# supernomad/quantum

Measured on AMD Instinct MI355X. Metric: AES-256-GCM seal+unseal GiB/s (device-resident packets) at 1/2/4/8 MI355X, higher is better.
Workload: dtype u8

## Files before the change

### quantum_amd/csrc/gcm_internal.h

```cpp
#pragma once
#include <hip/hip_runtime.h>

#include <sched.h>

#include <mutex>
#include <stdint.h>
#include <vector>

#include "../../include/qgcm.h"
#include "nonce_rng.h"
#include "one_fit.h"

namespace qgcm {

constexpr uint32_t kTeBytes = 65536;
constexpr uint32_t kGhBytes = 8192;
constexpr uint32_t kRkWords = 128;
constexpr uint32_t kGhEntries = 4608;
constexpr uint32_t kGhH = 0, kGhH4 = 512, kGhH2 = 1024, kGhH3 = 1536, kGhH5 = 2048;
constexpr uint32_t kGhH8 = 2560, kGhH16 = 3072, kGhH32 = 3584, kGhH64 = 4096;

struct Batch {
    uint8_t *arena;
    const qgcm_desc *descs;
    const uint32_t *worklist;
    const uint8_t *nonces;
    uint8_t *status;
    const uint32_t *rk_table;
    const uint4 *gh_table;
    const uint32_t *te;
    const uint8_t *key_valid;
    uint64_t stride;
    uint32_t uniform_len;
    uint32_t uniform_key;
    uint32_t n;
    uint32_t n_items;
    uint32_t aad_len;
    uint32_t max_keys;
    uint32_t *tile_counter;
    const uint32_t *tile_keys;
    const uint2 *runs;
    uint32_t *run_next;
    const uint32_t *nruns;
    const uint32_t *tile_list;
    const uint32_t *n_list;
    uint8_t *done;
    const uint4 *pw_table;
    uint32_t pw_keys;
    uint32_t *pool;
    uint32_t *pool_done;
    uint32_t pool_gen;
// ... 192 lines not shown
```

### quantum_amd/csrc/gcm_kernels.hip

```cpp
#include <hip/hip_runtime.h>
#include <stdint.h>

#include <algorithm>

#include "gcm_internal.h"

namespace qgcm {

typedef __attribute__((address_space(3))) uint32_t lds_u32;
typedef uint32_t u32x4 __attribute__((ext_vector_type(4)));
typedef __attribute__((address_space(3))) u32x4 lds_u128;

struct __attribute__((aligned(4))) W4 {
    uint32_t x, y, z, w;
};

#ifndef QGCM_NT_DATA
#define QGCM_NT_DATA 0
#endif
typedef uint32_t u32x4u __attribute__((ext_vector_type(4), aligned(4)));
__device__ __forceinline__ W4 load_block(const W4 *p) {
    if constexpr ((QGCM_NT_DATA & 1) != 0) {
        const u32x4u v = __builtin_nontemporal_load(reinterpret_cast<const u32x4u *>(p));
        return W4{v.x, v.y, v.z, v.w};
    }
    return *p;
}
__device__ __forceinline__ void store_block(W4 *p, const W4 &v) {
    if constexpr ((QGCM_NT_DATA & 2) != 0) {
        __builtin_nontemporal_store(u32x4u{v.x, v.y, v.z, v.w}, reinterpret_cast<u32x4u *>(p));
        return;
    }
    *p = v;
}

__device__ __forceinline__ uint32_t perm(uint32_t s0, uint32_t s1, uint32_t sel) {
// ... 135 lines not shown
    const uint32_t x = lo ^ c.x3;
    const uint32_t t0 = c.K0 ^ rot16(lds32(((x << 8) | t.lb) + kB + 128u));
    s0 = c.U0 ^ t.t0(t0, 0);
    s1 = c.U1 ^ rot16(t.t1(t0, 3));
    s2 = c.U2 ^ rot16(t.t0(t0, 2));
    s3 = c.U3 ^ t.t1(t0, 1);
#pragma unroll
    for (int r = 3; r < 14; ++r) round_full(s0, s1, s2, s3, k, r, t);
    round_last(s0, s1, s2, s3, k, t);
}
__device__ __forceinline__ void ctr_block(const Ctr &c, uint32_t lo, const Keys &k, uint32_t lb, uint32_t &s0,
                                          uint32_t &s1, uint32_t &s2, uint32_t &s3) {
    ctr_block_t<TT0, 0>(c, lo, k, TT0{lb, 0}, s0, s1, s2, s3);
}

template <bool kFence>
__device__ __forceinline__ void ghash_mul(uint32_t &y0, uint32_t &y1, uint32_t &y2, uint32_t &y3, uint32_t gb);

struct Tab2 {
    Keys kk;
    TT<0, true> t;
    __device__ __forceinline__ void setup(Ctr &c, uint32_t n0, uint32_t n1, uint32_t n2, uint32_t hi) const {
        ctr_setup(c, n0, n1, n2, hi, kk, t);
    }
    __device__ __forceinline__ void block(const Ctr &c, uint32_t lo, uint32_t &k0, uint32_t &k1, uint32_t &k2,
                                          uint32_t &k3) const {
        ctr_block_t<TT<0, true>, 0>(c, lo, kk, t, k0, k1, k2, k3);
    }
    __device__ __forceinline__ void ghash(uint32_t &y0, uint32_t &y1, uint32_t &y2, uint32_t &y3, uint32_t gb) const {
        ghash_mul<true>(y0, y1, y2, y3, gb);
    }
};

constexpr uint32_t kG5Windows = 26;
constexpr uint32_t kG5Bytes = kG5Windows * 512;

template <int kI>
__device__ __forceinline__ uint32_t g5_addr(const uint32_t (&y)[4], uint32_t mf8) {
    constexpr int p = 5 * kI, w = p >> 5, o = p & 31;
    uint32_t x;
    if constexpr (o > 27 && w < 3)
        x = __builtin_amdgcn_alignbit(y[w + 1], y[w], o - 3);
    else if constexpr (o > 3)
        x = y[w] >> (o - 3);
    else if constexpr (o < 3)
        x = y[w] << (3 - o);
    else
        x = y[w];
    return x & mf8;
}

template <int kLo, int kHi>
__device__ __forceinline__ void g5_chunk(const uint32_t (&y)[4], uint32_t mf8, uint32_t &a0, uint32_t &a1,
                                         uint32_t &a2, uint32_t &a3) {
    if constexpr (kLo < kHi) {
        if constexpr (QGCM_GH_PRIO > 0) __builtin_amdgcn_s_setprio(QGCM_GH_PRIO);
        const uint32_t x = g5_addr<kLo>(y, mf8);
        const u32x2 h0 = lds64(x + kLo * 512u), h1 = lds64(x + kLo * 512u + 256u);
        if constexpr (kLo + 1 < kHi) {
            const uint32_t x2 = g5_addr<kLo + 1>(y, mf8);
            const u32x2 l0 = lds64(x2 + (kLo + 1) * 512u), l1 = lds64(x2 + (kLo + 1) * 512u + 256u);
            if constexpr (QGCM_GH_PRIO > 0) __builtin_amdgcn_s_setprio(0);
            a0 = xor3(a0, h0.x, l0.x);
            a1 = xor3(a1, h0.y, l0.y);
            a2 = xor3(a2, h1.x, l1.x);
            a3 = xor3(a3, h1.y, l1.y);
            g5_chunk<kLo + 2, kHi>(y, mf8, a0, a1, a2, a3);
        } else {
            if constexpr (QGCM_GH_PRIO > 0) __builtin_amdgcn_s_setprio(0);
            a0 ^= h0.x;
            a1 ^= h0.y;
            a2 ^= h1.x;
            a3 ^= h1.y;
        }
    }
}

__device__ __forceinline__ void ghash_mul5(uint32_t &y0, uint32_t &y1, uint32_t &y2, uint32_t &y3, uint32_t mf8) {
    const uint32_t y[4] = {y0, y1, y2, y3};
    uint32_t a0 = 0, a1 = 0, a2 = 0, a3 = 0;
    g5_chunk<0, 7>(y, mf8, a0, a1, a2, a3);
    asm volatile("" : "+v"(a0), "+v"(a1), "+v"(a2), "+v"(a3)::"memory");
    g5_chunk<7, 13>(y, mf8, a0, a1, a2, a3);
    asm volatile("" : "+v"(a0), "+v"(a1), "+v"(a2), "+v"(a3)::"memory");
    g5_chunk<13, 20>(y, mf8, a0, a1, a2, a3);
    asm volatile("" : "+v"(a0), "+v"(a1), "+v"(a2), "+v"(a3)::"memory");
    g5_chunk<20, 26>(y, mf8, a0, a1, a2, a3);
    y0 = a0;
    y1 = a1;
    y2 = a2;
    y3 = a3;
}

__device__ __forceinline__ void g5_fill(const uint4 *__restrict__ comb4, uint32_t tid, uint32_t nthreads) {
    for (uint32_t e = tid; e < kG5Windows * 32u; e += nthreads) {
        const uint32_t i = e >> 5, v = e & 31u;
        uint4 c[5];
#pragma unroll
        for (uint32_t j = 0; j < 5; ++j) {
            const uint32_t t = 5 * i + j, tt = t < 128u ? t : 127u;
            const uint32_t vv = (((v >> j) & 1u) && t < 128u) ? (1u << (tt & 3u)) : 0u;
            c[j] = comb4[16u * (2u * (tt >> 3) + ((tt & 7u) < 4u ? 1u : 0u)) + vv];
        }
        uint32_t a0 = 0, a1 = 0, a2 = 0, a3 = 0;
#pragma unroll
        for (uint32_t j = 0; j < 5; ++j) {
            a0 ^= c[j].x;
            a1 ^= c[j].y;
            a2 ^= c[j].z;
            a3 ^= c[j].w;
        }
        *(lds_u64 *)(size_t)(512u * i + 8u * v) = u32x2{a0, a1};
        *(lds_u64 *)(size_t)(512u * i + 256u + 8u * v) = u32x2{a2, a3};
    }
}

struct Tab2F {
    Keys kk;
    TT<kG5Bytes, true> t;
    uint32_t mf8;
    __device__ __forceinline__ void setup(Ctr &c, uint32_t n0, uint32_t n1, uint32_t n2, uint32_t hi) const {
        ctr_setup(c, n0, n1, n2, hi, kk, t);
    }
    __device__ __forceinline__ void block(const Ctr &c, uint32_t lo, uint32_t &k0, uint32_t &k1, uint32_t &k2,
                                          uint32_t &k3) const {
        ctr_block_t<TT<kG5Bytes, true>, kG5Bytes>(c, lo, kk, t, k0, k1, k2, k3);
    }
    __device__ __forceinline__ void ghash(uint32_t &y0, uint32_t &y1, uint32_t &y2, uint32_t &y3, uint32_t) const {
        ghash_mul5(y0, y1, y2, y3, mf8);
    }
};

__device__ __forceinline__ uint32_t vreg(uint32_t x) {
    asm volatile("" : "+v"(x));
    return x;
}

template <bool kFence = true>
__device__ __forceinline__ void ghash_mul(uint32_t &y0, uint32_t &y1, uint32_t &y2, uint32_t &y3, uint32_t gb) {
    uint32_t a0 = 0, a1 = 0, a2 = 0, a3 = 0;
    const uint32_t yw[4] = {y0, y1, y2, y3};
#pragma unroll
    for (int w = 0; w < 4; ++w) {
        const uint32_t hi = yw[w] & 0xf0f0f0f0u;
        const uint32_t lo = (yw[w] << 4) & 0xf0f0f0f0u;
#pragma unroll
        for (int k = 0; k < 4; ++k) {
            const int j = 4 * w + k;
            const uint4 th = lds128(perm(gb, hi, 0x0c060500u | k) + (2 * j) * 256);
            const uint4 tl = lds128(perm(gb, lo, 0x0c060500u | k) + (2 * j + 1) * 256);
            a0 = xor3(a0, th.x, tl.x);
            a1 = xor3(a1, th.y, tl.y);
            a2 = xor3(a2, th.z, tl.z);
            a3 = xor3(a3, th.w, tl.w);
        }
        if constexpr (kFence) asm volatile("" : "+v"(a0), "+v"(a1), "+v"(a2), "+v"(a3)::"memory");
    }
    y0 = a0;
    y1 = a1;
    y2 = a2;
    y3 = a3;
}
// ... 232 lines not shown
    e2 = quad_xor(e2);
    e3 = quad_xor(e3);
    const uint32_t t0 = z0 ^ e0, t1 = z1 ^ e1, t2 = z2 ^ e2, t3 = z3 ^ e3;
    const uint32_t owner = r ? (nfull & 3u) : 0u;
    if (kSeal) {
        if (m == owner) {
            write_tail(data, L, t0, t1, t2, t3, n0, n1, n2, prefix);
            if (b.status) b.status[pkt] = 1;
        }
    } else {
        read_tag(data, L, g0, g1, g2, g3);
        const bool ok = ((t0 ^ g0) | (t1 ^ g1) | (t2 ^ g2) | (t3 ^ g3)) == 0;
        if (!ok) {
            for (uint32_t bi = m; bi < nfull; bi += 4) {
                const W4 zz = {0, 0, 0, 0};
                *reinterpret_cast<W4 *>(data + 16u * bi) = zz;
            }
            if (r && m == owner) {
                uint32_t *bw = reinterpret_cast<uint32_t *>(data + 16u * nfull);
                for (uint32_t w = 0; w < (r >> 2); ++w) bw[w] = 0;
                store_bytes(data + 16u * nfull + (r & ~3u), 0, r & 3u);
            }
        }
        if (b.status && m == 0) b.status[pkt] = ok ? 1 : 0;
    }
}

#ifndef QGCM_TILE_POOL
#define QGCM_TILE_POOL 4
#endif
#ifndef QGCM_TAIL_EIGHTHS
#define QGCM_TAIL_EIGHTHS 4
#endif
constexpr uint32_t kPoolCtr = kG5Bytes + kTeBytes;

#ifdef QGCM_QUAD_STATS
__device__ unsigned long long g_quad_stats[4096 * 8];
#endif

template <bool kDesc>
constexpr int quad_waves() { return kDesc ? 12 : 16; }
template <bool kDesc>
constexpr int quad_wpe() { return kDesc ? 3 : 8; }

template <bool kSeal, bool kDesc>
__global__ void __launch_bounds__(quad_waves<kDesc>() * 64) __attribute__((amdgpu_waves_per_eu(quad_wpe<kDesc>(),
                                                                                                  quad_wpe<kDesc>())))
gcm_quad_kernel(Batch b, const uint32_t *__restrict__ rk_table) {
    constexpr uint32_t kW = quad_waves<kDesc>();
    constexpr uint32_t kT = kW * 64;
    constexpr uint32_t kTeBase = kDesc ? 0u : kG5Bytes;
    const uint32_t lane = threadIdx.x & 63u;
    const uint32_t wave = threadIdx.x >> 6;
    const uint32_t m = lane & 3u;
    const uint32_t qd = lane >> 2;
    if (kDesc && b.tile_list && __builtin_amdgcn_readfirstlane(*b.n_list) == 0) return;

    for (uint32_t i = threadIdx.x; i < kTeBytes / 4; i += kT) {
        const uint32_t x = i >> 6, slot = i & 63u;
        lds_st32(kTeBase + 4 * i, b.te[(slot >> 5) * 256u + x]);
    }
    if constexpr (!kDesc) g5_fill(b.gh_table + (size_t)b.uniform_key * kGhEntries + kGhH4, threadIdx.x, kT);
    if constexpr (!kDesc && QGCM_TILE_POOL) {
        if (threadIdx.x == 0) lds_st32(kPoolCtr, kW);
    }
#if QGCM_TILE_POOL == 4
    if constexpr (!kDesc) {
        if (threadIdx.x == 0) lds_st32(kPoolCtr + 12, 0u);
    }
#endif
    __syncthreads();

    const uint32_t lb = (lane & 31u) << 2;
    const uint32_t m8 = vreg(0x0000ff00u), mf8 = vreg(0x000000f8u);
    const uint32_t gH4 = kDesc ? kTeBytes + wave * kGhBytes : 0u;
    uint32_t cur_key = kDesc ? 0xffffffffu : b.uniform_key;
    const uint32_t ntiles = kDesc ? (b.tile_list ? *b.n_list : b.n_items >> 4) : ((b.n + 15) >> 4);

#ifdef QGCM_QUAD_STATS
    unsigned long long *qs = g_quad_stats + (size_t)blockIdx.x * 8u;
    uint32_t qs_tiles = 0;
    if (!kDesc && threadIdx.x == 0) {
        qs[0] = wall_clock64();
        qs[4] = __builtin_amdgcn_s_getreg((31 << 11) | 20);
        qs[5] = __builtin_amdgcn_s_getreg((31 << 11) | 4);
    }
#endif
#ifdef QGCM_QUAD_STATS
#define QS_TILE() ++qs_tiles
#define QS_END()                                                  \
    do {                                                          \
        if (!kDesc && lane == 0) {                                \
            const unsigned long long t_ = wall_clock64();         \
            atomicMax(&qs[1], t_);                                \
            atomicAdd(&qs[2], t_);                                \
            atomicAdd(&qs[3], (unsigned long long)qs_tiles);      \
            atomicMax(&qs[6], (1ull << 62) - t_);                 \
        }                                                         \
    } while (0)
#else
#define QS_TILE() do { } while (0)
#define QS_END() do { } while (0)
#endif
#if QGCM_TILE_POOL == 4
    uint32_t sidx = 0xffffffffu, tail0 = 0;
    if constexpr (!kDesc) {
        const uint32_t rows = ntiles / (gridDim.x * kW);
// ... 52 lines not shown
            pkt = tile * 16u + qd;
            L = b.uniform_len;
            asm volatile("" : "+s"(L));
            valid = pkt < b.n;
            if (!kSeal) {
                if (L < (uint32_t)QGCM_OVERHEAD) valid = false;
                L -= QGCM_OVERHEAD;
            }
            off = (uint64_t)pkt * b.stride;
            if constexpr (QGCM_TILE_POOL) {
                uint32_t i = 0;
                if (lane == 0) i = __atomic_fetch_add((lds_u32 *)(size_t)kPoolCtr, 1u, __ATOMIC_RELAXED);
                i = __builtin_amdgcn_readfirstlane(i);
                tile = blockIdx.x * kW + (i % kW) + (i / kW) * gridDim.x * kW;
#if QGCM_TILE_POOL == 4
                if (i >= sidx) {
                    uint32_t c = 0;
                    if (lane == 0) c = atomicAdd(b.pool, 1u);
                    tile = tail0 + __builtin_amdgcn_readfirstlane(c);
                }
#endif
            } else {
                tile += gridDim.x * kW;
            }
            if (!valid) {
                if (!kSeal && b.status && pkt < b.n && m == 0) b.status[pkt] = 0;
                continue;
            }
        }
        const Keys kk = {rk_table + (size_t)wkey * kRkWords, rk_table + (size_t)wkey * kRkWords + 64};
        if constexpr (kDesc) {
            quad_packet<kSeal>(b, Tab2{kk, {lb, m8}}, pkt, off, L, wkey, m, gH4);
        } else {
            quad_packet<kSeal>(b, Tab2F{kk, {lb, m8}, mf8}, pkt, off, L, wkey, m, gH4);
        }
        QS_TILE();
    }
    QS_END();
#if QGCM_TILE_POOL == 4
    if constexpr (!kDesc) {
        if (b.pool) {
            uint32_t last = 0;
            if (lane == 0 && __atomic_fetch_add((lds_u32 *)(size_t)(kPoolCtr + 12), 1u, __ATOMIC_RELAXED) == kW - 1) {
                __threadfence();
                last = atomicAdd(b.pool + kPoolDoneWord, 1u) == gridDim.x - 1u ? 1u : 0u;
            }
            if (lane == 0 && last) {
                __threadfence();
                b.pool[0] = 0;
                b.pool[kPoolDoneWord] = 0;
                __threadfence_system();
                __hip_atomic_store(b.pool_done, b.pool_gen, __ATOMIC_RELEASE, __HIP_MEMORY_SCOPE_SYSTEM);
            }
        }
    }
#endif
}
#undef QS_TILE
#undef QS_END

#ifdef QGCM_QUAD_STATS
extern "C" int qgcm_debug_quad_stats(unsigned long long *out, int n, int reset) {
    if (n > 4096 * 8) n = 4096 * 8;
    if (hipMemcpyFromSymbol(out, HIP_SYMBOL(g_quad_stats), (size_t)n * 8) != hipSuccess) return -1;
    if (reset) {
        static unsigned long long zero[4096 * 8];
        if (hipMemcpyToSymbol(HIP_SYMBOL(g_quad_stats), zero, sizeof(zero)) != hipSuccess) return -1;
    }
    return 0;
}
#endif

constexpr uint32_t kSegCtl = kG5Bytes + kTeBytes;
constexpr uint32_t kSegLds = kSegCtl + 16u;
constexpr uint32_t kSegDone = 0xffffffffu;

__device__ __forceinline__ volatile lds_u32 *seg_ctl(uint32_t i) { return (volatile lds_u32 *)(size_t)(kSegCtl + 4u * i); }

template <class P>
__device__ __forceinline__ uint32_t wave_lower_bound(uint32_t lo, uint32_t hi, uint32_t lane, P pred) {
    while (hi - lo > 63u) {
        const uint32_t step = (hi - lo + 62u) / 63u;
        const uint32_t p = min(lo + lane * step, hi);
        const uint64_t msk = __ballot(pred(p));
        const uint32_t f = (uint32_t)__ffsll((unsigned long long)msk) - 1u;
        if (f == 0) return lo;
        const uint32_t nlo = lo + (f - 1u) * step + 1u, nhi = min(lo + f * step, hi);
        lo = nlo;
        hi = nhi;
    }
    const uint64_t msk = __ballot(pred(min(lo + lane, hi)));
    return lo + (uint32_t)__ffsll((unsigned long long)msk) - 1u;
}

#ifdef QGCM_SEG_STATS
__device__ unsigned long long g_seg_stats[4096 * 16];
#define SEG_STAT_ADD(i, v) \
    do { if (lane == 0) atomicAdd(&g_seg_stats[blockIdx.x * 16u + (i)], (unsigned long long)(v)); } while (0)
#define SEG_NOW() wall_clock64()
#else
#define SEG_STAT_ADD(i, v) do { } while (0)
#define SEG_NOW() 0ull
#endif

#ifndef QGCM_SEG_START
#define QGCM_SEG_START 1
// ... 43 lines not shown
            for (uint32_t j = 0; j < 4 && found == kSegDone; ++j) {
                const uint64_t msk = __ballot(left[j]);
                if (msk) found = __builtin_amdgcn_readfirstlane(__shfl(idx[j], (int)__ffsll((unsigned long long)msk) - 1));
            }
            if (found != kSegDone) break;
        }
    }
    uint32_t key = kSegDone;
    if (found != kSegDone) {
        r = found;
        key = b.tile_keys[b.runs[found].x];
    }
    if (lane == 0) {
        *seg_ctl(0) = found;
        *seg_ctl(1) = key;
    }
}

#ifndef QGCM_SEG_CLAIM
#define QGCM_SEG_CLAIM 1
#endif

template <bool kSeal>
__global__ void __launch_bounds__(1024) __attribute__((amdgpu_waves_per_eu(8, 8)))
gcm_seg_kernel(Batch b, const uint32_t *__restrict__ rk_table) {
    constexpr uint32_t kT = 1024;
    const uint32_t lane = threadIdx.x & 63u;
    const uint32_t wave = threadIdx.x >> 6;
    const uint32_t m = lane & 3u;
    const uint32_t qd = lane >> 2;
    if (__builtin_amdgcn_readfirstlane(*b.nruns) == 0) return;
    for (uint32_t i = threadIdx.x; i < kTeBytes / 4; i += kT) {
        const uint32_t x = i >> 6, slot = i & 63u;
        lds_st32(kG5Bytes + 4 * i, b.te[(slot >> 5) * 256u + x]);
    }
    const uint32_t lb = (lane & 31u) << 2;
    const uint32_t m8 = vreg(0x0000ff00u), mf8 = vreg(0x000000f8u);
    const uint32_t ntiles = b.n_items >> 4;
    uint32_t table_key = kSegDone;
    uint32_t r = 0, nruns = 0;
    bool helping = false;
    if (wave == 0) {
        nruns = *b.nruns;
        const uint32_t t = (uint32_t)((uint64_t)ntiles * blockIdx.x / gridDim.x);
        const uint32_t i = wave_lower_bound(0u, nruns, lane, [&](uint32_t j) { return j == nruns || b.runs[j].x > t; });
        r = i ? i - 1u : 0u;
        SEG_STAT_ADD(6, r);
        SEG_STAT_ADD(8, __builtin_amdgcn_s_getreg((31 << 11) | 20));
        SEG_STAT_ADD(9, __builtin_amdgcn_s_getreg((31 << 11) | 4));
    }
    __syncthreads();
    [[maybe_unused]] unsigned long long t_idle = SEG_NOW();
    if (wave == 0) SEG_STAT_ADD(2, t_idle);
    [[maybe_unused]] uint32_t ntile_stat = 0;
    for (;;) {
        if (wave == 0) {
            [[maybe_unused]] const unsigned long long t0 = SEG_NOW();
            seg_next_phase(b, r, nruns, helping, lane);
            SEG_STAT_ADD(7, SEG_NOW() - t0);
        }
        __syncthreads();
        if (wave == 0) SEG_STAT_ADD(0, 1);
        const uint32_t run = __builtin_amdgcn_readfirstlane(*seg_ctl(0));
        const uint32_t key = __builtin_amdgcn_readfirstlane(*seg_ctl(1));
        if (run == kSegDone) break;
        if (key != table_key) {
            g5_fill(b.gh_table + (size_t)key * kGhEntries + kGhH4, threadIdx.x, kT);
            table_key = key;
            __syncthreads();
        }
        [[maybe_unused]] const unsigned long long t_busy = SEG_NOW();
        SEG_STAT_ADD(4, t_busy - t_idle);
        const uint2 rt = b.runs[run];
        const Tab2F e3 = {{rk_table + (size_t)key * kRkWords, rk_table + (size_t)key * kRkWords + 64}, {lb, m8}, mf8};
        for (uint32_t t = 0, left = 0;; ++t, --left) {
            if (left == 0) {
                uint32_t nx = 0;
                if (lane == 0) nx = atomicAdd(b.run_next + run, (uint32_t)QGCM_SEG_CLAIM);
                t = rt.x + __builtin_amdgcn_readfirstlane(__shfl(nx, 0));
                left = QGCM_SEG_CLAIM;
            }
            if (t >= rt.y) break;
            const uint32_t pkt = b.worklist[t * 16u + qd];
            if (pkt != 0xffffffffu) {
                const qgcm_desc dsc = b.descs[pkt];
                const uint32_t L = kSeal ? dsc.len : dsc.len - QGCM_OVERHEAD;
                quad_packet<kSeal, Tab2F>(b, e3, pkt, dsc.offset, L, key, m, 0u);
            }
            ++ntile_stat;
        }
        t_idle = SEG_NOW();
        SEG_STAT_ADD(5, t_idle - t_busy);
        __syncthreads();
    }
    SEG_STAT_ADD(1, ntile_stat);
    if (wave == 0) SEG_STAT_ADD(3, SEG_NOW());
}

#ifdef QGCM_SEG_STATS
extern "C" int qgcm_debug_seg_stats(unsigned long long *out, int n, int reset) {
    if (n > 4096 * 16) n = 4096 * 16;
    if (hipMemcpyFromSymbol(out, HIP_SYMBOL(g_seg_stats), (size_t)n * 8) != hipSuccess) return -1;
    if (reset) {
        static unsigned long long zero[4096 * 16];
        if (hipMemcpyToSymbol(HIP_SYMBOL(g_seg_stats), zero, sizeof(zero)) != hipSuccess) return -1;
    }
    return 0;
}
#endif

constexpr uint32_t kOneThreads = 512;
constexpr uint32_t kOneTabs = 7;
constexpr uint32_t kOneBuf = kTeBytes + kOneTabs * kGhBytes;
constexpr uint32_t kOneScratch = kOneBuf + kOneCap;
constexpr uint32_t kOneX = kOneScratch + 64;
constexpr uint32_t kOneLds = kOneX + 2048;
constexpr uint32_t kOneSliceMax = kOneThreads / 4;
static_assert(kOneLds <= 160u * 1024u, "gfx950 LDS is 160 KiB per workgroup");
#ifdef QGCM_RES_TRACE
constexpr uint32_t kResTrace = ((kOneLds + 15u) & ~15u) + 16;
// ... 746 lines not shown
    if (b.aad_len > 4 && (b.n != 1 || b.descs || !one_fits_launch(b.uniform_len, seal, b.aad_len)))
        return hipErrorInvalidValue;
    if (!b.descs) {
        const uint64_t stage = (4ull + b.uniform_len + (seal ? QGCM_OVERHEAD : 0) + 15) & ~15ull;
        if ((b.n > 1 && (b.stride < stage || (b.stride & 15))) || stage > kOneCap - 16 ||
            (!seal && b.uniform_len < QGCM_OVERHEAD))
            return hipErrorInvalidValue;
    }
    void *args[] = {const_cast<Batch *>(&b), const_cast<uint32_t **>(&b.rk_table)};
    const void *k = seal ? reinterpret_cast<const void *>(&gcm_one_kernel<true>)
                         : reinterpret_cast<const void *>(&gcm_one_kernel<false>);
    return hipLaunchKernel(k, dim3(b.n), dim3(kOneThreads), args, kOneLds, s);
}

struct Variant {
    const void *seal, *open;
    int waves;
    uint32_t lds;
    int wgs_per_cu;
    bool desc;
    int complement;
};

static Variant g_variants[3];
static int variant_slot(int v) {
    return v == kVariantUniform ? 0 : v == kVariantDescWave ? 1 : v == kVariantDescQuad ? 2 : -1;
}

static const void *nonce_kernel_of(NonceDest dest);

hipError_t init_kernels() {
    g_variants[0] = Variant{reinterpret_cast<const void *>(&gcm_quad_kernel<true, false>),
                                          reinterpret_cast<const void *>(&gcm_quad_kernel<false, false>),
                                          quad_waves<false>(), kG5Bytes + kTeBytes + 16u,
                                          quad_wpe<false>() * 4 / quad_waves<false>(), false, -1};
    g_variants[1] = Variant{reinterpret_cast<const void *>(&gcm_quad_kernel<true, true>),
                                           reinterpret_cast<const void *>(&gcm_quad_kernel<false, true>),
                                           quad_waves<true>(), kTeBytes + (uint32_t)quad_waves<true>() * kGhBytes,
                                           1, true, -1};
    g_variants[2] = Variant{reinterpret_cast<const void *>(&gcm_seg_kernel<true>),
                                           reinterpret_cast<const void *>(&gcm_seg_kernel<false>), 16, kSegLds, 2, true,
                                           kVariantDescWave};
    for (const Variant &v : g_variants) {
        if (!v.seal) continue;
        for (const void *k : {v.seal, v.open}) {
            hipFuncAttributes a;
            hipError_t e = hipFuncGetAttributes(&a, k);
            if (e != hipSuccess) return e;
            if (a.sharedSizeBytes != 0) return hipErrorInvalidKernelFile;
            e = hipFuncSetAttribute(k, hipFuncAttributeMaxDynamicSharedMemorySize, v.lds);
            if (e != hipSuccess) return e;
        }
    }
    for (const void *k : {reinterpret_cast<const void *>(&gcm_one_kernel<true>),
                          reinterpret_cast<const void *>(&gcm_one_kernel<false>),
                          reinterpret_cast<const void *>(&gcm_resident_kernel)}) {
        hipFuncAttributes a;
        hipError_t e = hipFuncGetAttributes(&a, k);
        if (e != hipSuccess) return e;
        if (a.sharedSizeBytes != 0) return hipErrorInvalidKernelFile;
        e = hipFuncSetAttribute(k, hipFuncAttributeMaxDynamicSharedMemorySize,
                                k == reinterpret_cast<const void *>(&gcm_resident_kernel) ? kResLds : kOneLds);
        if (e != hipSuccess) return e;
    }
    for (NonceDest d : {kNonceArray, kNonceUniform, kNonceDescs}) {
        const void *k = nonce_kernel_of(d);
        hipFuncAttributes a;
// ... 17 lines not shown
    if (!variant_valid(variant)) return hipErrorInvalidValue;
    const Variant &v = g_variants[variant_slot(variant)];
    void *args[] = {const_cast<Batch *>(&b), const_cast<uint32_t **>(&b.rk_table)};
    return hipLaunchKernel(seal ? v.seal : v.open, dim3(grid), dim3(v.waves * 64), args, v.lds, s);
}

__device__ __forceinline__ uint8_t xt(uint8_t a) { return (uint8_t)((a << 1) ^ ((a & 0x80) ? 0x1b : 0)); }

__device__ inline void shift_x(uint8_t v[16]) {
    const int lsb = v[15] & 1;
    for (int j = 15; j > 0; --j) v[j] = (uint8_t)((v[j] >> 1) | (v[j - 1] << 7));
    v[0] >>= 1;
    if (lsb) v[0] ^= 0xe1;
}
__device__ inline uint4 pack16(const uint8_t v[16]) {
    uint4 w;
    w.x = v[0] | v[1] << 8 | v[2] << 16 | (uint32_t)v[3] << 24;
    w.y = v[4] | v[5] << 8 | v[6] << 16 | (uint32_t)v[7] << 24;
    w.z = v[8] | v[9] << 8 | v[10] << 16 | (uint32_t)v[11] << 24;
    w.w = v[12] | v[13] << 8 | v[14] << 16 | (uint32_t)v[15] << 24;
    return w;
}
__device__ inline void gf128_mul_bytes(const uint8_t X[16], const uint8_t Y[16], uint8_t Z[16]) {
    uint8_t z[16] = {0}, v[16];
    for (int i = 0; i < 16; ++i) v[i] = Y[i];
    for (int i = 0; i < 128; ++i) {
        if ((X[i >> 3] >> (7 - (i & 7))) & 1)
            for (int j = 0; j < 16; ++j) z[j] ^= v[j];
        shift_x(v);
    }
    for (int i = 0; i < 16; ++i) Z[i] = z[i];
}

__global__ void __launch_bounds__(256) key_setup_kernel(const uint8_t *keys, uint32_t first, uint32_t *rk_table,
                                                        uint4 *gh_table, const uint8_t *sbox_g) {
    __shared__ uint8_t sbox[256];
    __shared__ uint8_t rkb[240];
    constexpr int kT = kGhEntries / 512;
    __shared__ uint8_t hp[kT][16];
    __shared__ uint4 pw[kT][128];
    const uint32_t kidx = blockIdx.x;
    const uint8_t *key = keys + 32u * kidx;
    sbox[threadIdx.x] = sbox_g[threadIdx.x];
    __syncthreads();
    if (threadIdx.x == 0) {
        for (int i = 0; i < 32; ++i) rkb[i] = key[i];
        uint8_t rcon = 1;
        for (int i = 8; i < 60; ++i) {
            uint8_t t[4] = {rkb[4 * i - 4], rkb[4 * i - 3], rkb[4 * i - 2], rkb[4 * i - 1]};
            if (i % 8 == 0) {
                const uint8_t t0 = t[0];
                t[0] = sbox[t[1]] ^ rcon;
                t[1] = sbox[t[2]];
                t[2] = sbox[t[3]];
                t[3] = sbox[t0];
                rcon = xt(rcon);
            } else if (i % 8 == 4) {
                for (int j = 0; j < 4; ++j) t[j] = sbox[t[j]];
            }
            for (int j = 0; j < 4; ++j) rkb[4 * i + j] = rkb[4 * i - 32 + j] ^ t[j];
        }
        uint8_t s[16], u[16];
        for (int i = 0; i < 16; ++i) s[i] = rkb[i];
        for (int round = 1; round <= 14; ++round) {
            for (int c = 0; c < 4; ++c)
                for (int r = 0; r < 4; ++r) u[r + 4 * c] = sbox[s[r + 4 * ((c + r) & 3)]];
            if (round != 14) {
                for (int c = 0; c < 4; ++c) {
                    const uint8_t a0 = u[4 * c], a1 = u[4 * c + 1], a2 = u[4 * c + 2], a3 = u[4 * c + 3];
                    const uint8_t all = a0 ^ a1 ^ a2 ^ a3;
                    s[4 * c + 0] = a0 ^ all ^ xt(a0 ^ a1);
// ... 2 lines not shown
                    s[4 * c + 3] = a3 ^ all ^ xt(a3 ^ a0);
                }
            } else {
                for (int i = 0; i < 16; ++i) s[i] = u[i];
            }
            for (int i = 0; i < 16; ++i) s[i] ^= rkb[16 * round + i];
        }
        for (int i = 0; i < 16; ++i) hp[0][i] = s[i];
        gf128_mul_bytes(s, s, hp[2]);
        gf128_mul_bytes(hp[2], s, hp[3]);
        gf128_mul_bytes(hp[2], hp[2], hp[1]);
        gf128_mul_bytes(hp[1], s, hp[4]);
        for (int t = 5; t < kT; ++t) gf128_mul_bytes(hp[t == 5 ? 1 : t - 1], hp[t == 5 ? 1 : t - 1], hp[t]);
    }
    __syncthreads();
    if (threadIdx.x < kT) {
        uint8_t v[16];
        for (int i = 0; i < 16; ++i) v[i] = hp[threadIdx.x][i];
        for (int i = 0; i < 128; ++i) {
            pw[threadIdx.x][i] = pack16(v);
            shift_x(v);
        }
    }
    __syncthreads();
    const uint32_t slot = first + kidx;
    if (threadIdx.x < 64) {
        const int i = threadIdx.x;
        const uint32_t w = i < 60 ? (rkb[4 * i] | rkb[4 * i + 1] << 8 | rkb[4 * i + 2] << 16 |
                                     (uint32_t)rkb[4 * i + 3] << 24)
                                  : 0u;
        rk_table[(size_t)slot * kRkWords + i] = w;
        rk_table[(size_t)slot * kRkWords + 64 + i] = (w << 16) | (w >> 16);
    }
    for (uint32_t e = threadIdx.x; e < kGhEntries; e += 256) {
        const uint32_t p = (e & 511u) >> 4, v = e & 15u;
        const uint4 *src = pw[e >> 9];
        uint4 acc = {0, 0, 0, 0};
        for (int k = 0; k < 4; ++k) {
            if ((v >> (3 - k)) & 1u) {
                const uint4 t = src[4 * p + k];
                acc.x ^= t.x;
                acc.y ^= t.y;
                acc.z ^= t.z;
                acc.w ^= t.w;
            }
        }
        gh_table[(size_t)slot * kGhEntries + e] = acc;
    }
}

hipError_t launch_key_setup(const uint8_t *d_keys, uint32_t first, uint32_t count, uint32_t *rk_table,
                            uint4 *gh_table, const uint8_t *d_sbox, hipStream_t s) {
    if (count == 0) return hipSuccess;
    hipLaunchKernelGGL(key_setup_kernel, dim3(count), dim3(256), 0, s, d_keys, first, rk_table, gh_table, d_sbox);
    return hipGetLastError();
}

__global__ void __launch_bounds__(256) pw_setup_kernel(uint32_t first, const uint4 *gh_table, uint4 *pw,
                                                       uint32_t pw_keys) {
    __shared__ uint8_t hp[kPwPowers][16];
    __shared__ uint4 xs[16][128];
    const uint32_t slot = first + blockIdx.x, tid = threadIdx.x;
    if (slot >= pw_keys) return;
    if (tid == 0) {
        const uint4 h = gh_table[(size_t)slot * kGhEntries + kGhH + 8];
        const uint32_t w[4] = {h.x, h.y, h.z, h.w};
        for (int i = 0; i < 16; ++i) hp[0][i] = (uint8_t)(w[i >> 2] >> (8 * (i & 3)));
    }
    __syncthreads();
    for (uint32_t span = 1; span < kPwPowers; span <<= 1) {
        if (tid >= span && tid < 2 * span && tid < kPwPowers) gf128_mul_bytes(hp[tid - span], hp[span - 1], hp[tid]);
        __syncthreads();
    }
    for (uint32_t b0 = 0; b0 < kPwPowers; b0 += 16) {
        {
            const uint32_t j = tid >> 4, i0 = 8 * (tid & 15u);
            uint8_t v[16];
            for (int i = 0; i < 16; ++i) v[i] = hp[b0 + j][i];
            for (uint32_t i = 0; i < i0; ++i) shift_x(v);
            for (uint32_t i = 0; i < 8; ++i) {
// ... 211 lines not shown
```

### quantum_amd/csrc/qgcm_api.cpp

```cpp
#include <hip/hip_runtime.h>
#include <errno.h>
#include <stdint.h>
#include <stdio.h>
#include <stdlib.h>
#include <string.h>
#include <sys/random.h>

#include <algorithm>
#include <atomic>
#include <chrono>
#include <memory>
#include <future>
#include <map>
#include <mutex>
#include <thread>
#include <vector>

#include "../../include/qgcm.h"
#include "chain_claim.h"
#include "gcm_internal.h"
#include "kdf_core.h"

using namespace qgcm;

// ... 979 lines not shown
    const PeerPublics pp{priv_key, priv_salt, pub_keys, pub_salts};
    return derive_install_runs(ctx, &run, 1, count, nullptr, nullptr, &pp);
}

int qgcm_ecdh_stats(const qgcm_ctx *ctx, uint64_t *out, int n) {
    if (!ctx || !out || n < 0) return -1;
    const int m = std::min(n, 3);
    for (int i = 0; i < m; ++i) out[i] = ctx->ecdh_stats[i].load(std::memory_order_relaxed);
    return m;
}

int qgcm_kdf_stats(const qgcm_ctx *ctx, uint64_t *out, int n) {
    if (!ctx || !out || n < 0) return -1;
    const int m = std::min(n, 4);
    for (int i = 0; i < m; ++i) out[i] = ctx->kdf_stats[i].load(std::memory_order_relaxed);
    return m;
}

int qgcm_clear_keys(qgcm_ctx *ctx, uint32_t first_idx, uint32_t count) {
    if (!ctx) return QGCM_E_ARG;
    if ((uint64_t)first_idx + count > ctx->max_keys) return QGCM_E_KEY;
    if (count == 0) return QGCM_OK;
    if (hipSetDevice(ctx->device) != hipSuccess) return QGCM_E_HIP;
    std::lock_guard<std::mutex> io(ctx->io_mu);
    hipStream_t s = ctx->pipe[1];
    std::lock_guard<std::mutex> res_lk(ctx->res_mu);
    Resident *res = ctx->res.load(std::memory_order_acquire);
    (void)resident_pause(res);
    {
        std::lock_guard<std::mutex> g(ctx->key_mu);
        for (uint32_t i = 0; i < count; ++i) __atomic_store_n(&ctx->key_set[first_idx + i], (uint8_t)0, __ATOMIC_RELEASE);
    }
    int rc = QGCM_OK;
    if (hipMemsetAsync(ctx->d_key_valid + first_idx, 0, count, s) != hipSuccess || hipStreamSynchronize(s) != hipSuccess)
        rc = QGCM_E_HIP;
    resident_resume(res);
    return rc;
}

int qgcm_seal_batch(qgcm_ctx *ctx, uint8_t *d_arena, const qgcm_desc *d_descs, uint32_t n, const uint8_t *d_nonces,
                    uint32_t aad_len, uint8_t *d_status, void *stream) {
    return run_descs(ctx, true, d_arena, d_descs, n, d_nonces, aad_len, d_status, (hipStream_t)stream);
}

int qgcm_open_batch(qgcm_ctx *ctx, uint8_t *d_arena, const qgcm_desc *d_descs, uint32_t n, uint32_t aad_len,
                    uint8_t *d_status, void *stream) {
    return run_descs(ctx, false, d_arena, d_descs, n, nullptr, aad_len, d_status, (hipStream_t)stream);
}

int qgcm_seal_uniform(qgcm_ctx *ctx, uint8_t *d_arena, uint64_t stride, uint32_t n, uint32_t len, uint32_t key_idx,
                      const uint8_t *d_nonces, uint32_t aad_len, uint8_t *d_status, void *stream) {
    return run_uniform(ctx, true, d_arena, stride, n, len, key_idx, d_nonces, aad_len, d_status, (hipStream_t)stream);
}

int qgcm_open_uniform(qgcm_ctx *ctx, uint8_t *d_arena, uint64_t stride, uint32_t n, uint32_t len, uint32_t key_idx,
                      uint32_t aad_len, uint8_t *d_status, void *stream) {
    if (n > QGCM_MAX_BATCH) return QGCM_E_ARG;
    if (len < QGCM_OVERHEAD && n) {
        if (!ctx) return QGCM_E_ARG;
        if (d_status) {
            if (hipSetDevice(ctx->device) != hipSuccess) return QGCM_E_HIP;
            return hip_fail(hipMemsetAsync(d_status, 0, n, (hipStream_t)stream));
        }
        return QGCM_OK;
    }
    return run_uniform(ctx, false, d_arena, stride, n, len, key_idx, nullptr, aad_len, d_status, (hipStream_t)stream);
}
// ... 686 lines not shown
```

Measured before the change: 875.8.

## Serve upper GHASH 5-bit comb windows from global rows via buffer loads

Key setup now precomputes the 5-bit comb GHASH rows per key into the global gh_table. The uniform quad kernel then reads the top QGCM_GH_L1 windows (default 2) with buffer loads instead of LDS, interleaving those loads with the LDS lookups. This shrinks the LDS table, which may raise occupancy, and moves part of the lookup traffic to the L1/global path. In exchange each key's table grows by 13 KB, setup does more work, and clear_keys must also zero the extra rows.

```diff
diff --git a/quantum_amd/csrc/g5_comb.h b/quantum_amd/csrc/g5_comb.h
--- /dev/null
+++ b/quantum_amd/csrc/g5_comb.h
@@ -0,0 +1,30 @@
+#pragma once
+#include <stdint.h>
+
+#if defined(__HIPCC__) || defined(__CUDACC__)
+#define QGCM_G5_HD __host__ __device__
+#else
+#define QGCM_G5_HD
+#endif
+
+namespace qgcm {
+
+constexpr uint32_t kG5Windows = 26;
+constexpr uint32_t kG5Rows = kG5Windows * 32;
+
+QGCM_G5_HD constexpr uint32_t g5_bit_entry(uint32_t t) {
+    return 16u * (2u * (t >> 3) + ((t & 7u) < 4u ? 1u : 0u)) + (1u << (t & 3u));
+}
+
+QGCM_G5_HD constexpr uint32_t g5_term(uint32_t i, uint32_t v, uint32_t j) {
+    const uint32_t t = 5u * i + j, tt = t < 128u ? t : 127u;
+    return (((v >> j) & 1u) && t < 128u) ? g5_bit_entry(tt) : (g5_bit_entry(tt) & ~15u);
+}
+
+QGCM_G5_HD constexpr uint32_t g5_l1_first(uint32_t k) { return k >= 6u ? kG5Windows - k : 20u; }
+QGCM_G5_HD constexpr bool g5_in_l1(uint32_t i, uint32_t k) { return i >= g5_l1_first(k) && i < g5_l1_first(k) + k; }
+QGCM_G5_HD constexpr uint32_t g5_lds_slot(uint32_t i, uint32_t k) { return i < g5_l1_first(k) ? i : i - k; }
+QGCM_G5_HD constexpr uint32_t g5_lds_window(uint32_t slot, uint32_t k) { return slot < g5_l1_first(k) ? slot : slot + k; }
+QGCM_G5_HD constexpr uint32_t g5_lds_bytes(uint32_t k) { return (kG5Windows - k) * 512u; }
+
+}
diff --git a/quantum_amd/csrc/gcm_internal.h b/quantum_amd/csrc/gcm_internal.h
--- a/quantum_amd/csrc/gcm_internal.h
+++ b/quantum_amd/csrc/gcm_internal.h
@@ -8,6 +8,7 @@
 #include <vector>
 
 #include "../../include/qgcm.h"
+#include "g5_comb.h"
 #include "nonce_rng.h"
 #include "one_fit.h"
 
@@ -16,7 +17,9 @@
 constexpr uint32_t kTeBytes = 65536;
 constexpr uint32_t kGhBytes = 8192;
 constexpr uint32_t kRkWords = 128;
-constexpr uint32_t kGhEntries = 4608;
+constexpr uint32_t kGhComb = 4608;
+constexpr uint32_t kGhG5 = kGhComb;
+constexpr uint32_t kGhEntries = kGhComb + kG5Rows;
 constexpr uint32_t kGhH = 0, kGhH4 = 512, kGhH2 = 1024, kGhH3 = 1536, kGhH5 = 2048;
 constexpr uint32_t kGhH8 = 2560, kGhH16 = 3072, kGhH32 = 3584, kGhH64 = 4096;
 
diff --git a/quantum_amd/csrc/gcm_kernels.hip b/quantum_amd/csrc/gcm_kernels.hip
--- a/quantum_amd/csrc/gcm_kernels.hip
+++ b/quantum_amd/csrc/gcm_kernels.hip
@@ -2,6 +2,7 @@
 #include <stdint.h>
 
 #include <algorithm>
+#include <utility>
 
 #include "gcm_internal.h"
 
@@ -203,8 +204,64 @@
     }
 };
 
-constexpr uint32_t kG5Windows = 26;
-constexpr uint32_t kG5Bytes = kG5Windows * 512;
+#ifndef QGCM_GH_L1
+#define QGCM_GH_L1 2
+#endif
+#ifndef QGCM_GH_L1_SEG
+#define QGCM_GH_L1_SEG 0
+#endif
+static_assert(QGCM_GH_L1 >= 0 && QGCM_GH_L1 <= 12 && QGCM_GH_L1_SEG >= 0 && QGCM_GH_L1_SEG <= 12,
+              "windows served from the global rows: the upper windows, at most 12");
+constexpr uint32_t kGhL1 = QGCM_GH_L1, kGhL1Seg = QGCM_GH_L1_SEG;
+
+struct G5Rows {
+    __amdgpu_buffer_rsrc_t rsrc;
+};
+template <uint32_t kL1>
+__device__ __forceinline__ G5Rows g5_rows(const uint4 *gh_key) {
+    if constexpr (kL1 == 0) return G5Rows{};
+    const uint4 *rows = gh_key + kGhG5 + 32u * g5_l1_first(kL1);
+    return G5Rows{__builtin_amdgcn_make_buffer_rsrc(const_cast<uint4 *>(rows), 0, (int)(kL1 * 512u), 0x00020000)};
+}
+
+template <int kI>
+__device__ __forceinline__ uint32_t g5_row(const uint32_t (&y)[4]) {
+    constexpr int p = 5 * kI, w = p >> 5, o = p & 31;
+    uint32_t x;
+    if constexpr (o > 27 && w < 3)
+        x = __builtin_amdgcn_alignbit(y[w + 1], y[w], o - 4);
+    else if constexpr (o > 4)
+        x = y[w] >> (o - 4);
+    else if constexpr (o < 4)
+        x = y[w] << (4 - o);
+    else
+        x = y[w];
+    return x & 0x1f0u;
+}
+
+template <uint32_t kL1, uint32_t kLo, uint32_t... Q>
+__device__ __forceinline__ void g5_l1_issue(const uint32_t (&y)[4], const G5Rows &g, u32x4 *r,
+                                            std::integer_sequence<uint32_t, Q...>) {
+    ((r[Q] = __builtin_amdgcn_raw_buffer_load_b128(
+          g.rsrc, (int)(g5_row<(int)(g5_l1_first(kL1) + kLo + Q)>(y) + 512u * (kLo + Q)), 0, 0)),
+     ...);
+}
+template <uint32_t kN>
+__device__ __forceinline__ void g5_l1_add(const u32x4 *r, uint32_t &a0, uint32_t &a1, uint32_t &a2, uint32_t &a3) {
+#pragma unroll
+    for (uint32_t q = 0; q + 1 < kN; q += 2) {
+        a0 = xor3(a0, r[q].x, r[q + 1].x);
+        a1 = xor3(a1, r[q].y, r[q + 1].y);
+        a2 = xor3(a2, r[q].z, r[q + 1].z);
+        a3 = xor3(a3, r[q].w, r[q + 1].w);
+    }
+    if constexpr (kN & 1u) {
+        a0 ^= r[kN - 1].x;
+        a1 ^= r[kN - 1].y;
+        a2 ^= r[kN - 1].z;
+        a3 ^= r[kN - 1].w;
+    }
+}
 
 template <int kI>
 __device__ __forceinline__ uint32_t g5_addr(const uint32_t (&y)[4], uint32_t mf8) {
@@ -221,22 +278,22 @@
     return x & mf8;
 }
 
-template <int kLo, int kHi>
+template <uint32_t kL1, int kLo, int kHi>
 __device__ __forceinline__ void g5_chunk(const uint32_t (&y)[4], uint32_t mf8, uint32_t &a0, uint32_t &a1,
                                          uint32_t &a2, uint32_t &a3) {
     if constexpr (kLo < kHi) {
         if constexpr (QGCM_GH_PRIO > 0) __builtin_amdgcn_s_setprio(QGCM_GH_PRIO);
-        const uint32_t x = g5_addr<kLo>(y, mf8);
+        const uint32_t x = g5_addr<(int)g5_lds_window(kLo, kL1)>(y, mf8);
         const u32x2 h0 = lds64(x + kLo * 512u), h1 = lds64(x + kLo * 512u + 256u);
         if constexpr (kLo + 1 < kHi) {
-            const uint32_t x2 = g5_addr<kLo + 1>(y, mf8);
+            const uint32_t x2 = g5_addr<(int)g5_lds_window(kLo + 1, kL1)>(y, mf8);
             const u32x2 l0 = lds64(x2 + (kLo + 1) * 512u), l1 = lds64(x2 + (kLo + 1) * 512u + 256u);
             if constexpr (QGCM_GH_PRIO > 0) __builtin_amdgcn_s_setprio(0);
             a0 = xor3(a0, h0.x, l0.x);
             a1 = xor3(a1, h0.y, l0.y);
             a2 = xor3(a2, h1.x, l1.x);
             a3 = xor3(a3, h1.y, l1.y);
-            g5_chunk<kLo + 2, kHi>(y, mf8, a0, a1, a2, a3);
+            g5_chunk<kL1, kLo + 2, kHi>(y, mf8, a0, a1, a2, a3);
         } else {
             if constexpr (QGCM_GH_PRIO > 0) __builtin_amdgcn_s_setprio(0);
             a0 ^= h0.x;
@@ -247,32 +304,82 @@
     }
 }
 
-__device__ __forceinline__ void ghash_mul5(uint32_t &y0, uint32_t &y1, uint32_t &y2, uint32_t &y3, uint32_t mf8) {
+#ifndef QGCM_GH_L1_GROUP
+#define QGCM_GH_L1_GROUP 2
+#endif
+#ifndef QGCM_GH_L1_CHUNK
+#define QGCM_GH_L1_CHUNK 4
+#endif
+template <uint32_t kL1>
+struct G5Split {
+    static constexpr uint32_t kG = kL1 < QGCM_GH_L1_GROUP ? kL1 : QGCM_GH_L1_GROUP;
+    static constexpr uint32_t kLds = kG5Windows - kL1, kGroups = (kL1 + kG - 1) / kG;
+    static constexpr uint32_t kC = std::min<uint32_t>(QGCM_GH_L1_CHUNK, (kLds + kGroups - 1) / kGroups);
+    static constexpr uint32_t kChunks = (kLds + kC - 1) / kC;
+    static constexpr uint32_t kSteps = kGroups > kChunks ? kGroups : kChunks;
+};
+template <uint32_t kL1, uint32_t kS>
+__device__ __forceinline__ void g5_lds_chunks(const uint32_t (&y)[4], uint32_t mf8, uint32_t &a0, uint32_t &a1,
+                                              uint32_t &a2, uint32_t &a3) {
+    using S = G5Split<kL1>;
+    if constexpr (kS < S::kChunks) {
+        g5_chunk<kL1, (int)(kS * S::kC), (int)std::min(S::kLds, (kS + 1) * S::kC)>(y, mf8, a0, a1, a2, a3);
+        asm volatile("" : "+v"(a0), "+v"(a1), "+v"(a2), "+v"(a3)::"memory");
+        g5_lds_chunks<kL1, kS + 1>(y, mf8, a0, a1, a2, a3);
+    }
+}
+template <uint32_t kL1, uint32_t kS>
+__device__ __forceinline__ void g5_steps(const uint32_t (&y)[4], uint32_t mf8, const G5Rows &g, uint32_t &a0,
+                                         uint32_t &a1, uint32_t &a2, uint32_t &a3) {
+    using S = G5Split<kL1>;
+    if constexpr (kS < S::kSteps) {
+        constexpr uint32_t lo = kS * S::kG, cnt = lo < kL1 ? std::min(S::kG, kL1 - lo) : 0u;
+        u32x4 r[S::kG];
+        if constexpr (cnt > 0) g5_l1_issue<kL1, lo>(y, g, r, std::make_integer_sequence<uint32_t, cnt>{});
+        if constexpr (kS < S::kChunks) {
+            g5_chunk<kL1, (int)(kS * S::kC), (int)std::min(S::kLds, (kS + 1) * S::kC)>(y, mf8, a0, a1, a2, a3);
+            asm volatile("" : "+v"(a0), "+v"(a1), "+v"(a2), "+v"(a3)::"memory");
+        }
+        if constexpr (cnt > 0) g5_l1_add<cnt>(r, a0, a1, a2, a3);
+        g5_steps<kL1, kS + 1>(y, mf8, g, a0, a1, a2, a3);
+    }
+}
+
+template <uint32_t kL1>
+__device__ __forceinline__ void ghash_mul5(uint32_t &y0, uint32_t &y1, uint32_t &y2, uint32_t &y3, uint32_t mf8,
+                                           const G5Rows &g) {
     const uint32_t y[4] = {y0, y1, y2, y3};
     uint32_t a0 = 0, a1 = 0, a2 = 0, a3 = 0;
-    g5_chunk<0, 7>(y, mf8, a0, a1, a2, a3);
-    asm volatile("" : "+v"(a0), "+v"(a1), "+v"(a2), "+v"(a3)::"memory");
-    g5_chunk<7, 13>(y, mf8, a0, a1, a2, a3);
-    asm volatile("" : "+v"(a0), "+v"(a1), "+v"(a2), "+v"(a3)::"memory");
-    g5_chunk<13, 20>(y, mf8, a0, a1, a2, a3);
-    asm volatile("" : "+v"(a0), "+v"(a1), "+v"(a2), "+v"(a3)::"memory");
-    g5_chunk<20, 26>(y, mf8, a0, a1, a2, a3);
+    if constexpr (kL1 == 0) {
+        g5_chunk<0, 0, 7>(y, mf8, a0, a1, a2, a3);
+        asm volatile("" : "+v"(a0), "+v"(a1), "+v"(a2), "+v"(a3)::"memory");
+        g5_chunk<0, 7, 13>(y, mf8, a0, a1, a2, a3);
+        asm volatile("" : "+v"(a0), "+v"(a1), "+v"(a2), "+v"(a3)::"memory");
+        g5_chunk<0, 13, 20>(y, mf8, a0, a1, a2, a3);
+        asm volatile("" : "+v"(a0), "+v"(a1), "+v"(a2), "+v"(a3)::"memory");
+        g5_chunk<0, 20, 26>(y, mf8, a0, a1, a2, a3);
+    } else if constexpr (G5Split<kL1>::kGroups == 1) {
+        u32x4 r[kL1];
+        g5_l1_issue<kL1, 0>(y, g, r, std::make_integer_sequence<uint32_t, kL1>{});
+        asm volatile("" ::: "memory");
+        g5_lds_chunks<kL1, 0>(y, mf8, a0, a1, a2, a3);
+        g5_l1_add<kL1>(r, a0, a1, a2, a3);
+    } else {
+        g5_steps<kL1, 0>(y, mf8, g, a0, a1, a2, a3);
+    }
     y0 = a0;
     y1 = a1;
     y2 = a2;
     y3 = a3;
 }
 
+template <uint32_t kL1>
 __device__ __forceinline__ void g5_fill(const uint4 *__restrict__ comb4, uint32_t tid, uint32_t nthreads) {
-    for (uint32_t e = tid; e < kG5Windows * 32u; e += nthreads) {
-        const uint32_t i = e >> 5, v = e & 31u;
+    for (uint32_t e = tid; e < (kG5Windows - kL1) * 32u; e += nthreads) {
+        const uint32_t blk = e >> 5, i = g5_lds_window(blk, kL1), v = e & 31u;
         uint4 c[5];
 #pragma unroll
-        for (uint32_t j = 0; j < 5; ++j) {
-            const uint32_t t = 5 * i + j, tt = t < 128u ? t : 127u;
-            const uint32_t vv = (((v >> j) & 1u) && t < 128u) ? (1u << (tt & 3u)) : 0u;
-            c[j] = comb4[16u * (2u * (tt >> 3) + ((tt & 7u) < 4u ? 1u : 0u)) + vv];
-        }
+        for (uint32_t j = 0; j < 5; ++j) c[j] = comb4[g5_term(i, v, j)];
         uint32_t a0 = 0, a1 = 0, a2 = 0, a3 = 0;
 #pragma unroll
         for (uint32_t j = 0; j < 5; ++j) {
@@ -281,24 +388,27 @@
             a2 ^= c[j].z;
             a3 ^= c[j].w;
         }
-        *(lds_u64 *)(size_t)(512u * i + 8u * v) = u32x2{a0, a1};
-        *(lds_u64 *)(size_t)(512u * i + 256u + 8u * v) = u32x2{a2, a3};
-    }
-}
-
+        *(lds_u64 *)(size_t)(512u * blk + 8u * v) = u32x2{a0, a1};
+        *(lds_u64 *)(size_t)(512u * blk + 256u + 8u * v) = u32x2{a2, a3};
+    }
+}
+
+template <uint32_t kL1>
 struct Tab2F {
+    static constexpr uint32_t kTe = g5_lds_bytes(kL1);
     Keys kk;
-    TT<kG5Bytes, true> t;
+    TT<kTe, true> t;
     uint32_t mf8;
+    G5Rows rows;
     __device__ __forceinline__ void setup(Ctr &c, uint32_t n0, uint32_t n1, uint32_t n2, uint32_t hi) const {
         ctr_setup(c, n0, n1, n2, hi, kk, t);
     }
     __device__ __forceinline__ void block(const Ctr &c, uint32_t lo, uint32_t &k0, uint32_t &k1, uint32_t &k2,
                                           uint32_t &k3) const {
-        ctr_block_t<TT<kG5Bytes, true>, kG5Bytes>(c, lo, kk, t, k0, k1, k2, k3);
+        ctr_block_t<TT<kTe, true>, kTe>(c, lo, kk, t, k0, k1, k2, k3);
     }
     __device__ __forceinline__ void ghash(uint32_t &y0, uint32_t &y1, uint32_t &y2, uint32_t &y3, uint32_t) const {
-        ghash_mul5(y0, y1, y2, y3, mf8);
+        ghash_mul5<kL1>(y0, y1, y2, y3, mf8, rows);
     }
 };
 
@@ -597,7 +707,7 @@
 #ifndef QGCM_TAIL_EIGHTHS
 #define QGCM_TAIL_EIGHTHS 4
 #endif
-constexpr uint32_t kPoolCtr = kG5Bytes + kTeBytes;
+constexpr uint32_t kPoolCtr = g5_lds_bytes(kGhL1) + kTeBytes;
 
 #ifdef QGCM_QUAD_STATS
 __device__ unsigned long long g_quad_stats[4096 * 8];
@@ -614,7 +724,7 @@
 gcm_quad_kernel(Batch b, const uint32_t *__restrict__ rk_table) {
     constexpr uint32_t kW = quad_waves<kDesc>();
     constexpr uint32_t kT = kW * 64;
-    constexpr uint32_t kTeBase = kDesc ? 0u : kG5Bytes;
+    constexpr uint32_t kTeBase = kDesc ? 0u : g5_lds_bytes(kGhL1);
     const uint32_t lane = threadIdx.x & 63u;
     const uint32_t wave = threadIdx.x >> 6;
     const uint32_t m = lane & 3u;
@@ -625,7 +735,7 @@
         const uint32_t x = i >> 6, slot = i & 63u;
         lds_st32(kTeBase + 4 * i, b.te[(slot >> 5) * 256u + x]);
     }
-    if constexpr (!kDesc) g5_fill(b.gh_table + (size_t)b.uniform_key * kGhEntries + kGhH4, threadIdx.x, kT);
+    if constexpr (!kDesc) g5_fill<kGhL1>(b.gh_table + (size_t)b.uniform_key * kGhEntries + kGhH4, threadIdx.x, kT);
     if constexpr (!kDesc && QGCM_TILE_POOL) {
         if (threadIdx.x == 0) lds_st32(kPoolCtr, kW);
     }
@@ -638,6 +748,7 @@
 
     const uint32_t lb = (lane & 31u) << 2;
     const uint32_t m8 = vreg(0x0000ff00u), mf8 = vreg(0x000000f8u);
+    [[maybe_unused]] const G5Rows rows = g5_rows<kDesc ? 0u : kGhL1>(b.gh_table + (size_t)b.uniform_key * kGhEntries);
     const uint32_t gH4 = kDesc ? kTeBytes + wave * kGhBytes : 0u;
     uint32_t cur_key = kDesc ? 0xffffffffu : b.uniform_key;
     const uint32_t ntiles = kDesc ? (b.tile_list ? *b.n_list : b.n_items >> 4) : ((b.n + 15) >> 4);
@@ -756,7 +867,7 @@
         if constexpr (kDesc) {
             quad_packet<kSeal>(b, Tab2{kk, {lb, m8}}, pkt, off, L, wkey, m, gH4);
         } else {
-            quad_packet<kSeal>(b, Tab2F{kk, {lb, m8}, mf8}, pkt, off, L, wkey, m, gH4);
+            quad_packet<kSeal>(b, Tab2F<kGhL1>{kk, {lb, m8}, mf8, rows}, pkt, off, L, wkey, m, gH4);
         }
         QS_TILE();
     }
@@ -795,7 +906,7 @@
 }
 #endif
 
-constexpr uint32_t kSegCtl = kG5Bytes + kTeBytes;
+constexpr uint32_t kSegCtl = g5_lds_bytes(kGhL1Seg) + kTeBytes;
 constexpr uint32_t kSegLds = kSegCtl + 16u;
 constexpr uint32_t kSegDone = 0xffffffffu;
 
@@ -905,7 +1016,7 @@
     if (__builtin_amdgcn_readfirstlane(*b.nruns) == 0) return;
     for (uint32_t i = threadIdx.x; i < kTeBytes / 4; i += kT) {
         const uint32_t x = i >> 6, slot = i & 63u;
-        lds_st32(kG5Bytes + 4 * i, b.te[(slot >> 5) * 256u + x]);
+        lds_st32(g5_lds_bytes(kGhL1Seg) + 4 * i, b.te[(slot >> 5) * 256u + x]);
     }
     const uint32_t lb = (lane & 31u) << 2;
     const uint32_t m8 = vreg(0x0000ff00u), mf8 = vreg(0x000000f8u);
@@ -938,14 +1049,15 @@
         const uint32_t key = __builtin_amdgcn_readfirstlane(*seg_ctl(1));
         if (run == kSegDone) break;
         if (key != table_key) {
-            g5_fill(b.gh_table + (size_t)key * kGhEntries + kGhH4, threadIdx.x, kT);
+            g5_fill<kGhL1Seg>(b.gh_table + (size_t)key * kGhEntries + kGhH4, threadIdx.x, kT);
             table_key = key;
             __syncthreads();
         }
         [[maybe_unused]] const unsigned long long t_busy = SEG_NOW();
         SEG_STAT_ADD(4, t_busy - t_idle);
         const uint2 rt = b.runs[run];
-        const Tab2F e3 = {{rk_table + (size_t)key * kRkWords, rk_table + (size_t)key * kRkWords + 64}, {lb, m8}, mf8};
+        const Tab2F<kGhL1Seg> e3 = {{rk_table + (size_t)key * kRkWords, rk_table + (size_t)key * kRkWords + 64}, {lb, m8}, mf8,
+                                    g5_rows<kGhL1Seg>(b.gh_table + (size_t)key * kGhEntries)};
         for (uint32_t t = 0, left = 0;; ++t, --left) {
             if (left == 0) {
                 uint32_t nx = 0;
@@ -958,7 +1070,7 @@
             if (pkt != 0xffffffffu) {
                 const qgcm_desc dsc = b.descs[pkt];
                 const uint32_t L = kSeal ? dsc.len : dsc.len - QGCM_OVERHEAD;
-                quad_packet<kSeal, Tab2F>(b, e3, pkt, dsc.offset, L, key, m, 0u);
+                quad_packet<kSeal, Tab2F<kGhL1Seg>>(b, e3, pkt, dsc.offset, L, key, m, 0u);
             }
             ++ntile_stat;
         }
@@ -1771,7 +1883,7 @@
 hipError_t init_kernels() {
     g_variants[0] = Variant{reinterpret_cast<const void *>(&gcm_quad_kernel<true, false>),
                                           reinterpret_cast<const void *>(&gcm_quad_kernel<false, false>),
-                                          quad_waves<false>(), kG5Bytes + kTeBytes + 16u,
+                                          quad_waves<false>(), kPoolCtr + 16u,
                                           quad_wpe<false>() * 4 / quad_waves<false>(), false, -1};
     g_variants[1] = Variant{reinterpret_cast<const void *>(&gcm_quad_kernel<true, true>),
                                            reinterpret_cast<const void *>(&gcm_quad_kernel<false, true>),
@@ -1855,11 +1967,26 @@
     for (int i = 0; i < 16; ++i) Z[i] = z[i];
 }
 
+__device__ inline uint4 comb4_entry(const uint4 *pw, uint32_t e) {
+    const uint32_t p = e >> 4, v = e & 15u;
+    uint4 acc = {0, 0, 0, 0};
+    for (int k = 0; k < 4; ++k) {
+        if ((v >> (3 - k)) & 1u) {
+            const uint4 t = pw[4 * p + k];
+            acc.x ^= t.x;
+            acc.y ^= t.y;
+            acc.z ^= t.z;
+            acc.w ^= t.w;
+        }
+    }
+    return acc;
+}
+
 __global__ void __launch_bounds__(256) key_setup_kernel(const uint8_t *keys, uint32_t first, uint32_t *rk_table,
                                                         uint4 *gh_table, const uint8_t *sbox_g) {
     __shared__ uint8_t sbox[256];
     __shared__ uint8_t rkb[240];
-    constexpr int kT = kGhEntries / 512;
+    constexpr int kT = kGhComb / 512;
     __shared__ uint8_t hp[kT][16];
     __shared__ uint4 pw[kT][128];
     const uint32_t kidx = blockIdx.x;
@@ -1928,20 +2055,18 @@
         rk_table[(size_t)slot * kRkWords + i] = w;
         rk_table[(size_t)slot * kRkWords + 64 + i] = (w << 16) | (w >> 16);
     }
-    for (uint32_t e = threadIdx.x; e < kGhEntries; e += 256) {
-        const uint32_t p = (e & 511u) >> 4, v = e & 15u;
-        const uint4 *src = pw[e >> 9];
+    for (uint32_t e = threadIdx.x; e < kGhComb; e += 256)
+        gh_table[(size_t)slot * kGhEntries + e] = comb4_entry(pw[e >> 9], e & 511u);
+    for (uint32_t r = threadIdx.x; r < kG5Rows; r += 256) {
         uint4 acc = {0, 0, 0, 0};
-        for (int k = 0; k < 4; ++k) {
-            if ((v >> (3 - k)) & 1u) {
-                const uint4 t = src[4 * p + k];
-                acc.x ^= t.x;
-                acc.y ^= t.y;
-                acc.z ^= t.z;
-                acc.w ^= t.w;
-            }
-        }
-        gh_table[(size_t)slot * kGhEntries + e] = acc;
+        for (uint32_t j = 0; j < 5; ++j) {
+            const uint4 t = comb4_entry(pw[kGhH4 >> 9], g5_term(r >> 5, r & 31u, j));
+            acc.x ^= t.x;
+            acc.y ^= t.y;
+            acc.z ^= t.z;
+            acc.w ^= t.w;
+        }
+        gh_table[(size_t)slot * kGhEntries + kGhG5 + r] = acc;
     }
 }
 
diff --git a/quantum_amd/csrc/qgcm_api.cpp b/quantum_amd/csrc/qgcm_api.cpp
--- a/quantum_amd/csrc/qgcm_api.cpp
+++ b/quantum_amd/csrc/qgcm_api.cpp
@@ -1035,7 +1035,10 @@
         for (uint32_t i = 0; i < count; ++i) __atomic_store_n(&ctx->key_set[first_idx + i], (uint8_t)0, __ATOMIC_RELEASE);
     }
     int rc = QGCM_OK;
-    if (hipMemsetAsync(ctx->d_key_valid + first_idx, 0, count, s) != hipSuccess || hipStreamSynchronize(s) != hipSuccess)
+    if (hipMemsetAsync(ctx->d_key_valid + first_idx, 0, count, s) != hipSuccess ||
+        hipMemset2DAsync(ctx->d_gh + (size_t)first_idx * kGhEntries + kGhG5, (size_t)kGhEntries * 16, 0, (size_t)kG5Rows * 16,
+                         count, s) != hipSuccess ||
+        hipStreamSynchronize(s) != hipSuccess)
         rc = QGCM_E_HIP;
     resident_resume(res);
     return rc;
```

New measurement: 879.5 (median of 6 runs). No clear change (+0.4%).
